# TheCacophonyProject/classifier-pipeline

Hardware: AMD Instinct MI355X
Metric: CPTV frames/s end-to-end (track+classify) at 160x120 (higher is better)
Workload: dtype u16/i32 track stage (f32 normalise, f64 gates); f32 crop/tile; f32 CNN (stride-1 3x3 convs of stages 2-4 (+ the stride-2 one): two fp16 planes per operand rounded to nearest (11 + 11 significand bits), power-of-two range scaling, 3 fp16 MFMAs per K step, device-side rerun in the exact split if an ac

## Files before the change

### classifier-pipeline_amd/csrc/cpx_api.cpp

```cpp
#include <hip/hip_runtime.h>

#include <algorithm>
#include <cmath>
#include <cstdio>
#include <cstdlib>
#include <cstring>
#include <new>
#include <string>
#include <vector>

#include "cpx_internal.h"
#include "cpx_schedule_core.h"

static_assert(sizeof(cpx_component) == 32, "cpx_component layout is part of the ABI");
static_assert(sizeof(cpx_frame_info) == 80, "cpx_frame_info layout is part of the ABI");
static_assert(sizeof(cpx_frame_meta) == 24, "cpx_frame_meta layout is part of the ABI");
static_assert(sizeof(cpx_config) == 48, "cpx_config layout is part of the ABI");
static_assert(sizeof(cpx_region_ref) == 24 && sizeof(cpx_track_limits) == 32 && sizeof(cpx_crop_req) == 32,
              "classification request layouts are part of the ABI");
static_assert(sizeof(cpx_filter_params) == 72 && sizeof(cpx_track_summary) == 120,
              "end-of-clip layouts are part of the ABI");
static_assert(sizeof(cpx_region) == 56, "cpx_region layout is part of the ABI");
static_assert(sizeof(cpx_track_record) == 32, "cpx_track_record layout is part of the ABI");
static_assert(sizeof(cpx_track_params) == 120, "cpx_track_params layout is part of the ABI");
// ... 100 lines not shown
    }
    if (lut[63] != 0 || h->nlm_lut_dev.grow(h, 64 * sizeof(int), "NLM weight table allocation") ||
        hipMemcpy(h->nlm_lut_dev.p, lut.data(), 64 * sizeof(int), hipMemcpyHostToDevice) != hipSuccess) {
      cpx_destroy(h);
      return CPX_ERR_HIP;
    }
  }
  std::vector<uint32_t> thr(h->wtab_len);
  for (int k = 0; k < h->wtab_len; ++k) {
    const double wk = wt[k], m = std::nearbyint(wk);
    const bool exact = (wk == m), near = !exact && std::fabs(wk - m) < 1e-6;
    double hi = near ? m + 1.0 : std::floor(wk) + 1.0;
    if (!(hi >= 0.0)) hi = 0.0;
    if (hi > 536870912.0) hi = 536870912.0;
    thr[k] = 2u * (uint32_t)hi - (near ? 1u : 0u);
  }
  if (h->wthr_dev.grow(h, thr.size() * sizeof(uint32_t), "threshold table allocation") ||
      hipMemcpy(h->wthr_dev.p, thr.data(), thr.size() * sizeof(uint32_t), hipMemcpyHostToDevice) != hipSuccess) {
    cpx_destroy(h);
    return CPX_ERR_HIP;
  }
  if (h->wtab_dev.grow(h, wt.size() * sizeof(double), "weight table allocation") ||
      hipMemcpy(h->wtab_dev.p, wt.data(), wt.size() * sizeof(double), hipMemcpyHostToDevice) != hipSuccess ||
      cpx::frame_kernel_attr_setup() != 0) {
    cpx_destroy(h);
    return CPX_ERR_HIP;
  }
  if (const char* env = std::getenv("CPX_TRACK_PACKED_STATE")) h->packed_state_ok = std::atoi(env) != 0;
  if (const char* env = std::getenv("CPX_CNN_FUSE_CONV1")) h->fuse_conv1 = std::atoi(env) != 0;
  if (const char* env = std::getenv("CPX_TRACK_PER_STEP")) h->track_per_step = std::atoi(env) != 0;
  if (const char* env = std::getenv("CPX_CNN_FUSE_SHORTCUT")) h->fuse_shortcut = std::atoi(env) != 0;
  if (const char* env = std::getenv("CPX_CNN_SHORTCUT_FP16")) h->shortcut_fp16 = std::atoi(env) != 0;
  if (const char* env = std::getenv("CPX_CNN_FLAT16")) h->flat16 = std::atoi(env) != 0;
  if (const char* env = std::getenv("CPX_CNN_BLOCK_FUSION")) h->block_fusion = std::min(std::max(std::atoi(env), 0), 2);
  if (const char* env = std::getenv("CPX_CNN_MATH")) {
    if (!std::strcmp(env, "f32")) h->cnn_math = CPX_CNN_MATH_F32;
    else if (!std::strcmp(env, "bf16x3")) h->cnn_math = CPX_CNN_MATH_BF16X3;
    else if (!std::strcmp(env, "bf16x2")) h->cnn_math = CPX_CNN_MATH_BF16X2;
    else if (!std::strcmp(env, "fp16x2")) h->cnn_math = CPX_CNN_MATH_FP16X2;
  }
  *out = h;
  return CPX_OK;
}

static void release_buffers(cpx_handle* h, bool all) {
  for (DeviceBuffer* b : {&h->ws, &h->ws_assoc, &h->bf3_scratch, &h->cnn_arena, &h->graph_arena, &h->ir_scratch}) b->release();
  if (!all) return;
  for (DeviceBuffer* b : {&h->sched, &h->wtab_dev, &h->wthr_dev, &h->nlm_lut_dev, &h->cnn_ovf, &h->ir_bitmap}) b->release();
}

void cpx_destroy(cpx_handle* h) {
  if (!h) return;
  hipSetDevice(h->device);
  if (h->stream) hipStreamSynchronize(h->stream);
  for (cpx_cnn* c : h->cnns) cnn_free(c);
  h->cnns.clear();
  for (cpx_mog2* m : h->mog2s) mog2_free(m);
  h->mog2s.clear();
  for (cpx_graph* g : h->graphs) graph_free(g);
  h->graphs.clear();
  release_buffers(h, true);
  for (auto& e : h->conv_events) {
    hipEventDestroy(e.e0);
    hipEventDestroy(e.e1);
  }
  if (h->stream2) {
// ... 731 lines not shown
```

### classifier-pipeline_amd/csrc/cpx_api_cnn.cpp

```cpp
#include <hip/hip_runtime.h>

#include <algorithm>
#include <cmath>
#include <cstdio>
#include <cstdlib>
#include <new>
#include <utility>
#include <vector>

#include "cpx_internal.h"

static_assert(sizeof(cpx_wrresnet_block) == 56 && sizeof(cpx_wrresnet_params) == 1560,
              "cpx_wrresnet_params layout is part of the ABI");

struct cpx_cnn {
  cpx_handle* h = nullptr;
  cpx_wrresnet_params p{};
  std::vector<std::pair<const float*, void*>> split;
  float act_scale[3][CPX_WRRESNET_MAX_BLOCKS][2];
  float res_bound[3] = {0.0f, 0.0f, 0.0f};
  float sc_xscale[3] = {0.0f, 0.0f, 0.0f};
  void* sc_img[3] = {nullptr, nullptr, nullptr};
  double sc_wmax[3] = {-1.0, -1.0, -1.0};
  cpx_cnn() {
// ... 123 lines not shown
  const conv_half& k = hf ? *hf : bare;
  const bool fp16 = split && h->cnn_math == CPX_CNN_MATH_FP16X2;
  const bool aliased = a.out == a.residual || a.out == a.in;
  const bool half = fp16 && cpx::conv_bf3_two_planes(a) && !aliased;
  const bool planes_out = fp16 && k.out_planes;
  const ConvRoute route = k.rerun_only ? ConvRoute::RerunOnly
                          : !split ? ConvRoute::Float32
                          : (half || planes_out) ? ConvRoute::Fp16Pair
                                                 : ConvRoute::Split;
  ConvTimer timer(h, h->conv_timing && route != ConvRoute::RerunOnly);
  if (!timer.ok()) return fail(h, CPX_ERR_HIP, "cpx_conv2d: event creation failed");
  int* word = nullptr;
  if (route == ConvRoute::Fp16Pair || route == ConvRoute::RerunOnly) {
    if (int rc = ensure_ovf_word(h)) return rc;
    if (!k.keep_flag) CPX_HIP(h, hipMemsetAsync(h->cnn_ovf.p, 0, sizeof(int), h->stream));
    word = h->cnn_ovf.as<int>() + k.word;
  }
  if (split && !split_weights) {
    if (int rc = h->bf3_scratch.grow(h, cpx::conv_bf3_weight_bytes(a), "cpx_conv2d: weight scratch allocation failed"))
      return rc;
    cpx::launch_split_weights(a, h->bf3_scratch.p, h->stream);
    split_weights = h->bf3_scratch.p;
  }
  int rc = 0;
  if (route == ConvRoute::Fp16Pair) {
    cpx::ConvArgs first = a;
    if (half) {
      first.planes = 2;
      first.half = 1;
      first.act_scale = k.act_scale;
      first.act_unscale = 1.0f / first.act_scale;
      first.in_planes = k.in_planes;
      first.flat16 = h->flat16;
    }
    first.ovf = word;
    if (planes_out) {
      first.out_planes = 1;
      first.out_act_scale = k.out_act_scale;
    }
    rc = cpx::launch_conv_bf3(first, split_weights, h->stream);
  }
  a.guard = word;
  if (split) {
    if (rc == 0) rc = cpx::launch_conv_bf3(a, split_weights, h->stream);
    if (rc == -3) {
      if (fuse) return fail(h, CPX_ERR_UNSUPPORTED, "conv_run: batch too large for the fused-shortcut kernel (split the call)");
      rc = cpx::launch_conv(a, h->stream);
    }
  } else {
    rc = cpx::launch_conv(a, h->stream);
  }
  if (int trc = timer.commit((a.Cin / a.groups) * 10000 + (a.Cout / a.groups) * 10 + a.stride + (a.ksize == 1 ? 5 : 0),
                             2.0 * a.N * a.Ho * a.Wo * a.Cout * (double)(a.Cin / a.groups) * a.ksize * a.ksize))
    return trc;
  if (rc == -2) return fail(h, CPX_ERR_UNSUPPORTED, "cpx_conv2d: no kernel for this (channels per group, stride, kernel size)");
  if (rc != 0) return fail(h, CPX_ERR_HIP, "cpx_conv2d: kernel configuration failed");
  CPX_HIP(h, hipGetLastError());
  return CPX_OK;
}

static bool conv_can_fuse(const cpx_handle* h, int f, int groups) {
  return split_math(h) && cpx::conv_bf3_supported(conv_shape(0, 0, 0, f, f, groups, 3, 1, 1));
}

enum class BlockForm {
  OneLaunch,
// ... 557 lines not shown
```

### classifier-pipeline_amd/csrc/cpx_cnn_rw.hip

```cpp
#include <hip/hip_runtime.h>

#include <algorithm>
#include <type_traits>

#include "cpx_cnn_dev.h"
#include "cpx_conv_layout_core.h"
#include "cpx_kernels.h"

namespace cpx {

namespace {

struct RwTiles : Tiles {};

constexpr int RW_TW = 16;
constexpr int RW_CT = 256;
constexpr int RW_PPI = RW_CT / 8;
constexpr int RW_WC = 64;

template <int S, int NCH, int ROWS>
struct RwGeo {
  static constexpr int PW = 15 * S + 3, PH = (ROWS - 1) * S + 3, NPX = PH * PW;
  static constexpr int NP = (NPX * 8 + RW_CT - 1) / RW_CT;
  static constexpr int NPXP = (NP * RW_PPI + 3) / 4 * 4 + 2;
  static constexpr int BUF = 2 * 2 * NPXP * 2;
  static constexpr int STEPS = 3 * PH;
  static constexpr int CING = 32 * NCH;
  static constexpr size_t LDS = (size_t)2 * BUF * 16 + (size_t)(2 * CING + 3 * RW_WC) * sizeof(float);
};
constexpr int SC_NPXP = 258;
constexpr int SC_ITEMS = 16 * RW_TW * 8 / RW_CT;
constexpr size_t SC_LDS = (size_t)2 * 2 * SC_NPXP * 2 * 16;

template <int S, int NCH, int ROWS, bool BN, bool RES, bool SC = false>
__global__ __launch_bounds__(RW_CT) __attribute__((amdgpu_waves_per_eu(1, 1))) void conv_rw_kernel(ConvArgs a, const uint4* __restrict__ wimg, RwTiles td) {
  using G = RwGeo<S, NCH, ROWS>;
  constexpr int PW = G::PW, NPX = G::NPX, NP = G::NP, NPXP = G::NPXP, BUF = G::BUF, STEPS = G::STEPS, CING = G::CING, PH = G::PH;
  static_assert(!SC || (S == 1 && NCH == 2 && ROWS == 16 && !RES), "the fp16 shortcut is built into the stride-1 form's two-chunk stream");
  if (*a.ovf != 0) return;
  extern __shared__ __attribute__((aligned(16))) uint4 lds4[];
  uint4* s_buf = lds4;
  float* s_bn = reinterpret_cast<float*>(lds4 + 2 * BUF);
  float* s_par = s_bn + 2 * CING;
  uint4* s_sc = reinterpret_cast<uint4*>(s_par + 3 * RW_WC);
  const int tid = threadIdx.x, lane = tid & 63, wave = tid >> 6, i16 = lane & 15, q = lane >> 4;
  const int ct = wave;
  const int cout_g = a.Cout / a.groups, nhalf = cout_g / RW_WC;
  const int g = blockIdx.y / nhalf, half = blockIdx.y - g * nhalf;
  constexpr bool has_bn = BN;

  u32x4 Wr[NCH][9][2];
  {
    const u32x4* wg = reinterpret_cast<const u32x4*>(wimg) + (size_t)g * NCH * 3 * 24 * cout_g + (q * cout_g + half * RW_WC + ct * 16 + i16);
#pragma unroll
    for (int c = 0; c < NCH; ++c)
#pragma unroll
      for (int ky = 0; ky < 3; ++ky)
#pragma unroll
        for (int kx = 0; kx < 3; ++kx)
#pragma unroll
          for (int p = 0; p < 2; ++p) Wr[c][ky * 3 + kx][p] = wg[(size_t)((c * 3 + ky) * 24 + (p * 3 + kx) * 4) * cout_g];
  }
  u32x4 Wsc[2];
  if constexpr (SC) {
    const u32x4* ws = reinterpret_cast<const u32x4*>(a.sc_planes) + (size_t)g * 8 * cout_g + (q * cout_g + half * RW_WC + ct * 16 + i16);
    Wsc[0] = ws[0];
    Wsc[1] = ws[(size_t)4 * cout_g];
  }
  if (tid < CING) {
    const int ci = g * CING + tid;
    s_bn[tid] = has_bn ? a.in_scale[ci] * a.act_scale : a.act_scale;
    s_bn[CING + tid] = has_bn ? a.in_shift[ci] * a.act_scale : 0.0f;
  }
  if (tid < RW_WC) {
    const int ch = g * cout_g + half * RW_WC + tid;
    float os = a.w_unscale[ch] * a.act_unscale;
    if (a.out_scale) os *= a.out_scale[ch];
    float ob = a.out_shift ? a.out_shift[ch] : 0.0f;
    if (a.sc_in && a.sc_bias) ob += a.sc_bias[ch];
    s_par[tid] = os;
    s_par[RW_WC + tid] = ob;
    s_par[2 * RW_WC + tid] = a.w_scale[ch] * a.act_scale;
  }

  const int per_xcd = (td.total + 7) >> 3;
  auto tile_of = [&](int t) { return (t & 7) * per_xcd + (t >> 3); };
  auto decode = [&](int tile, int& n_, int& oy_, int& ox_) {
    int qd = tile_div(tile, td.m_tx);
    ox_ = (tile - qd * td.tiles_x) * RW_TW;
    tile = qd;
    qd = tile_div(tile, td.m_ty);
    oy_ = (tile - qd * td.tiles_y) * ROWS;
    n_ = qd;
  };
  int t = blockIdx.x;
  while (t < 8 * per_xcd && tile_of(t) >= td.total) t += gridDim.x;
  if (t >= 8 * per_xcd) return;
  auto advance = [&](int& n_, int& oy_, int& ox_) {
    t += gridDim.x;
    const bool more = t < 8 * per_xcd && tile_of(t) < td.total;
    if (more) decode(tile_of(t), n_, oy_, ox_);
    return more;
  };
  int n0, oy0, ox0, n1, oy1, ox1, n2, oy2, ox2;
  decode(tile_of(t), n0, oy0, ox0);

  u32x4 pre_p[NP];
  const int q8 = tid & 7;
  int ipos[NP];
#pragma unroll
  for (int i = 0; i < NP; ++i) {
    const int px = min((tid >> 3) + RW_PPI * i, NPX - 1);
    const int py = px / PW;
    ipos[i] = (py << 8) | (px - py * PW);
  }
  const unsigned st_base = (unsigned)((((q8 >> 2) * NPXP + (tid >> 3)) * 4 + (q8 & 3)) * 8);
  f32x4 psc[NCH], psh[NCH];
  const unsigned coff0 = (unsigned)(g * CING + 4 * q8);
  const int Hm1 = a.H - 1, Wm1 = a.W - 1;
  auto issue_item = [&](const int i, const int c, const int n_, const int oy_, const int ox_) __attribute__((always_inline)) {
    const float* in_n = a.in + (size_t)n_ * a.H * a.W * a.Cin;
    const int iy = oy_ * S - a.pad_top + (ipos[i] >> 8), ix = ox_ * S - a.pad_left + (ipos[i] & 0xFF);
    const int cy = med3(iy, 0, Hm1), cx = med3(ix, 0, Wm1);
    pre_p[i] = *reinterpret_cast<const u32x4*>(at_off(in_n, (pix_off(cy, cx, a.W, a.Cin) + coff0 + (unsigned)(c * 32)) << 2));
  };
  unsigned hmax = 0u;
  auto activate_item = [&](const int i, const int c, const int oy_, const int ox_) __attribute__((always_inline)) {
    float v[4];
#pragma unroll
    for (int j = 0; j < 4; ++j) v[j] = __fmaf_rn(__uint_as_float(pre_p[i][j]), psc[c][j], psh[c][j]);
    if (has_bn) {
#pragma unroll
      for (int j = 0; j < 4; ++j) v[j] = fmaxf(v[j], 0.0f);
    }
    const int iy = oy_ * S - a.pad_top + (ipos[i] >> 8), ix = ox_ * S - a.pad_left + (ipos[i] & 0xFF);
    const bool inside = (unsigned)iy < (unsigned)a.H && (unsigned)ix < (unsigned)a.W;
#pragma unroll
    for (int j = 0; j < 4; ++j) pre_p[i][j] = __float_as_uint(inside ? v[j] : 0.0f);
  };
  auto store_item = [&](const int i, const int bsel) __attribute__((always_inline)) {
    unsigned h0, h1, l0, l1;
    split_pair2_h(__uint_as_float(pre_p[i][0]), __uint_as_float(pre_p[i][1]), h0, l0);
    split_pair2_h(__uint_as_float(pre_p[i][2]), __uint_as_float(pre_p[i][3]), h1, l1);
    if (has_bn) hmax = pk_max_u16(pk_max_u16(hmax, h0), h1);
    else hmax = pk_max_u16(pk_max_u16(hmax, h0 & 0x7FFF7FFFu), h1 & 0x7FFF7FFFu);
    unsigned char* sp = reinterpret_cast<unsigned char*>(s_buf) + st_base;
    *reinterpret_cast<uint2*>(sp + (bsel * BUF * 16 + i * (RW_PPI * 32))) = make_uint2(h0, h1);
    *reinterpret_cast<uint2*>(sp + (bsel * BUF * 16 + 2 * NPXP * 32 + i * (RW_PPI * 32))) = make_uint2(l0, l1);
  };

  u32x4 pre_s[SC ? SC_ITEMS : 1];
  u32x4 xsh[2], xsl[2];
  const unsigned sc_st_base = (unsigned)((((q8 >> 2) * SC_NPXP + (tid >> 3)) * 4 + (q8 & 3)) * 8);
  const int sc_a_base = ((q >> 1) * SC_NPXP + i16) * 2 + (q & 1);
  auto issue_sc = [&](const int i, const int n_, const int oy_, const int ox_) __attribute__((always_inline)) {
    if constexpr (SC) {
      const float* sc_n = a.sc_in + (size_t)n_ * a.sc_H * a.sc_W * a.sc_cin;
      const int oy = min(oy_ + 2 * i + (tid >> 7), a.Ho - 1), ox = min(ox_ + ((tid >> 3) & 15), a.Wo - 1);
      pre_s[i] = *reinterpret_cast<const u32x4*>(
          at_off(sc_n, (pix_off(oy * a.sc_stride, ox * a.sc_stride, a.sc_W, a.sc_cin) + (unsigned)(g * 32 + 4 * q8)) << 2));
    }
  };
  auto store_sc = [&](const int i) __attribute__((always_inline)) {
    if constexpr (SC) {
      unsigned h0, h1, l0, l1;
      split_pair2_h(__uint_as_float(pre_s[i][0]) * a.sc_xscale, __uint_as_float(pre_s[i][1]) * a.sc_xscale, h0, l0);
      split_pair2_h(__uint_as_float(pre_s[i][2]) * a.sc_xscale, __uint_as_float(pre_s[i][3]) * a.sc_xscale, h1, l1);
      hmax = pk_max_u16(pk_max_u16(hmax, h0 & 0x7FFF7FFFu), h1 & 0x7FFF7FFFu);
      unsigned char* sp = reinterpret_cast<unsigned char*>(s_sc) + sc_st_base;
      *reinterpret_cast<uint2*>(sp + i * (RW_PPI * 32)) = make_uint2(h0, h1);
      *reinterpret_cast<uint2*>(sp + (2 * SC_NPXP * 32 + i * (RW_PPI * 32))) = make_uint2(l0, l1);
    }
  };

  f32x4 acc[ROWS];
  const int ch_l = g * cout_g + half * RW_WC + ct * 16 + 4 * q;
  auto init_acc = [&]() __attribute__((always_inline)) {
#pragma unroll
    for (int o = 0; o < ROWS; ++o) acc[o] = f32x4{0.0f, 0.0f, 0.0f, 0.0f};
  };
  f32x4 rres[RES ? ROWS : 1];
  auto issue_res = [&](const int o, const int n_, const int oy_, const int ox_) __attribute__((always_inline)) {
    if constexpr (RES) {
      const float* res_n = a.residual + (size_t)n_ * a.Ho * a.Wo * a.Cout;
      const int ox = min(ox_ + i16, a.Wo - 1), oy = min(oy_ + o, a.Ho - 1);
      rres[o] = *reinterpret_cast<const f32x4*>(at_off(res_n, (pix_off(oy, ox, a.Wo, a.Cout) + (unsigned)ch_l) << 2));
    }
  };

  const int a_base = ((q >> 1) * NPXP + S * i16) * 2 + (q & 1);
  constexpr int RW_AHEAD = 3, RW_RING = RW_AHEAD + 1;
  auto compute = [&](auto cc, auto bc, auto&& between) __attribute__((always_inline)) {
    constexpr int C = decltype(cc)::value, B = decltype(bc)::value;
    const uint4* sb = s_buf + B * BUF + a_base;
    u32x4 xh[RW_RING], xl[RW_RING];
    auto frag = [&](auto sc) __attribute__((always_inline)) {
      constexpr int s = decltype(sc)::value;
      constexpr int kx = s / PH, i = s - PH * kx, bf = s % RW_RING;
      xh[bf] = __builtin_bit_cast(u32x4, sb[(i * PW + kx) * 2]);
      xl[bf] = __builtin_bit_cast(u32x4, sb[4 * NPXP + (i * PW + kx) * 2]);
    };
    static_for<0, RW_AHEAD>(frag);
    static_for<0, STEPS>([&](auto sc) __attribute__((always_inline)) {
      constexpr int s = decltype(sc)::value;
      constexpr int kx = s / PH, i = s - PH * kx, bf = s % RW_RING;
      if constexpr (s + RW_AHEAD < STEPS) frag(std::integral_constant<int, s + RW_AHEAD>{});
      static_for<0, 3>([&](auto pc) __attribute__((always_inline)) {
        constexpr int pr = decltype(pc)::value;
        static_for<0, 3>([&](auto rc) __attribute__((always_inline)) {
          constexpr int r = decltype(rc)::value, d = i - r, o = d / S;
          if constexpr (d >= 0 && d % S == 0 && o < ROWS) {
            if constexpr (pr == 0) acc[o] = mfma16<true>(Wr[C][r * 3 + kx][1], xh[bf], acc[o]);
            if constexpr (pr == 1) acc[o] = mfma16<true>(Wr[C][r * 3 + kx][0], xl[bf], acc[o]);
            if constexpr (pr == 2) acc[o] = mfma16<true>(Wr[C][r * 3 + kx][0], xh[bf], acc[o]);
          }
        });
      });
      between(sc);
      __builtin_amdgcn_sched_barrier(0);
    });
  };
  auto unit = [&](auto cc, auto bc, auto ccc, auto cic, auto lastc, const int oyc, const int oxc, const int ni, const int oyi,
                  const int oxi) __attribute__((always_inline)) {
    constexpr int B = decltype(bc)::value, CC = decltype(ccc)::value, CI = decltype(cic)::value;
    constexpr bool LAST = decltype(lastc)::value;
    compute(cc, bc, [&](auto sc) __attribute__((always_inline)) {
      constexpr int s = decltype(sc)::value;
      constexpr int jlo = (s * 3 * NP + STEPS - 1) / STEPS, jhi = ((s + 1) * 3 * NP + STEPS - 1) / STEPS;
      static_for<jlo, (jhi < 3 * NP ? jhi : 3 * NP)>([&](auto jc) __attribute__((always_inline)) {
        constexpr int j = decltype(jc)::value, i = j / 3, k = j % 3;
        if constexpr (k == 0) activate_item(i, CC, oyc, oxc);
        if constexpr (k == 1) store_item(i, B ^ 1);
        if constexpr (k == 2) issue_item(i, CI, ni, oyi, oxi);
      });
      if constexpr (SC && !LAST) {
        constexpr int klo = (s * SC_ITEMS + STEPS - 1) / STEPS, khi = ((s + 1) * SC_ITEMS + STEPS - 1) / STEPS;
        static_for<klo, (khi < SC_ITEMS ? khi : SC_ITEMS)>([&](auto kc) __attribute__((always_inline)) { store_sc(decltype(kc)::value); });
      }
      if constexpr (SC && LAST) {
        if constexpr (s % 3 == 0 && s >= 3 && s / 3 - 1 < ROWS) {
          constexpr int o = s / 3 - 1;
          acc[o] = mfma16<true>(Wsc[1], xsh[o & 1], acc[o]);
          acc[o] = mfma16<true>(Wsc[0], xsl[o & 1], acc[o]);
          acc[o] = mfma16<true>(Wsc[0], xsh[o & 1], acc[o]);
        }
        if constexpr (s % 3 == 0 && s / 3 < ROWS) {
          constexpr int o = s / 3;
          xsh[o & 1] = __builtin_bit_cast(u32x4, s_sc[sc_a_base + o * 2 * RW_TW]);
          xsl[o & 1] = __builtin_bit_cast(u32x4, s_sc[sc_a_base + 4 * SC_NPXP + o * 2 * RW_TW]);
        }
        constexpr int klo = (s * SC_ITEMS + STEPS - 1) / STEPS, khi = ((s + 1) * SC_ITEMS + STEPS - 1) / STEPS;
        static_for<klo, (khi < SC_ITEMS ? khi : SC_ITEMS)>([&](auto kc) __attribute__((always_inline)) { issue_sc(decltype(kc)::value, ni, oyi, oxi); });
      }
      if constexpr (LAST && RES) {
        constexpr int olo = (s * ROWS + STEPS - 1) / STEPS, ohi = ((s + 1) * ROWS + STEPS - 1) / STEPS;
        static_for<olo, (ohi < ROWS ? ohi : ROWS)>([&](auto oc) __attribute__((always_inline)) { issue_res(decltype(oc)::value, n0, oy0, ox0); });
      }
    });
  };

  auto finish = [&](const int n_, const int oy_, const int ox_) __attribute__((always_inline)) {
    const int ox = min(ox_ + i16, a.Wo - 1);
    if (!SC && a.sc_in) {
      const int sc_cg = a.sc_cin / a.groups;
      const float* wsc = a.sc_w + ((size_t)g * sc_cg + q) * cout_g + half * RW_WC + ct * 16 + i16;
      const float ss = s_par[2 * RW_WC + ct * 16 + i16];
      const float* sc_n = a.sc_in + (size_t)n_ * a.sc_H * a.sc_W * a.sc_cin + g * sc_cg + q;
      for (int k4 = 0; k4 < sc_cg; k4 += 4) {
        const float ws = wsc[(size_t)k4 * cout_g] * ss;
#pragma unroll
        for (int o = 0; o < ROWS; ++o) {
          const int oy = min(oy_ + o, a.Ho - 1);
          const float xs = sc_n[((size_t)(oy * a.sc_stride) * a.sc_W + ox * a.sc_stride) * a.sc_cin + k4];
          acc[o] = __builtin_amdgcn_mfma_f32_16x16x4f32(ws, xs, acc[o], 0, 0, 0);
        }
      }
    }
    float* out_n = a.out + (size_t)n_ * a.Ho * a.Wo * a.Cout;
    const f32x4 os = *reinterpret_cast<const f32x4*>(s_par + ct * 16 + 4 * q);
    const f32x4 ob = *reinterpret_cast<const f32x4*>(s_par + RW_WC + ct * 16 + 4 * q);
    const bool xok = ox_ + i16 < a.Wo;
    const unsigned off0 = (pix_off(min(oy_, a.Ho - 1), ox, a.Wo, a.Cout) + (unsigned)ch_l) << 2;
    const unsigned row_bytes = (unsigned)(a.Wo * a.Cout) << 2;
    const bool whole = oy_ + ROWS <= a.Ho;
    auto row = [&](const int o, const bool ok, const unsigned off) __attribute__((always_inline)) {
      f32x4 v;
#pragma unroll
      for (int j = 0; j < 4; ++j) v[j] = __fmaf_rn(acc[o][j], os[j], ob[j]);
      if constexpr (RES) v += rres[o];
      if (a.relu) {
        asm volatile("");
        v.x = relu_bits(v.x); v.y = relu_bits(v.y); v.z = relu_bits(v.z); v.w = relu_bits(v.w);
      }
      if (ok) *reinterpret_cast<f32x4*>(at_off(out_n, off)) = v;
    };
    if (whole) {
#pragma unroll
      for (int o = 0; o < ROWS; ++o) row(o, xok, off0 + (unsigned)o * row_bytes);
    } else {
#pragma unroll
      for (int o = 0; o < ROWS; ++o) row(o, xok && oy_ + o < a.Ho, off0 + (unsigned)min(o, a.Ho - 1 - oy_) * row_bytes);
    }
  };

#pragma unroll
  for (int i = 0; i < NP; ++i) issue_item(i, 0, n0, oy0, ox0);
  __syncthreads();
#pragma unroll
  for (int c = 0; c < NCH; ++c) {
    psc[c] = *reinterpret_cast<const f32x4*>(s_bn + c * 32 + 4 * q8);
    psh[c] = *reinterpret_cast<const f32x4*>(s_bn + CING + c * 32 + 4 * q8);
  }
#pragma unroll
  for (int i = 0; i < NP; ++i) {
    activate_item(i, 0, oy0, ox0);
    store_item(i, 0);
  }
  using I0 = std::integral_constant<int, 0>;
  using I1 = std::integral_constant<int, 1>;
  using Yes = std::integral_constant<bool, true>;
  using No = std::integral_constant<bool, false>;
  if constexpr (NCH == 2) {
#pragma unroll
    for (int i = 0; i < NP; ++i) issue_item(i, 1, n0, oy0, ox0);
    if constexpr (SC) {
#pragma unroll
      for (int i = 0; i < SC_ITEMS; ++i) issue_sc(i, n0, oy0, ox0);
    }
    init_acc();
    for (;;) {
      n1 = n0; oy1 = oy0; ox1 = ox0;
      const bool more = advance(n1, oy1, ox1);
      __syncthreads();
      unit(I0{}, I0{}, I1{}, I0{}, No{}, oy0, ox0, n1, oy1, ox1);
      __syncthreads();
      unit(I1{}, I1{}, I0{}, I1{}, Yes{}, oy1, ox1, n1, oy1, ox1);
      finish(n0, oy0, ox0);
      if (!more) break;
      n0 = n1; oy0 = oy1; ox0 = ox1;
      init_acc();
    }
  } else {
    n1 = n0; oy1 = oy0; ox1 = ox0;
    bool more1 = advance(n1, oy1, ox1);
#pragma unroll
    for (int i = 0; i < NP; ++i) issue_item(i, 0, n1, oy1, ox1);
    init_acc();
    for (;;) {
      n2 = n1; oy2 = oy1; ox2 = ox1;
      bool more2 = more1 && advance(n2, oy2, ox2);
      __syncthreads();
      unit(I0{}, I0{}, I0{}, I0{}, Yes{}, oy1, ox1, n2, oy2, ox2);
      finish(n0, oy0, ox0);
      if (!more1) break;
      n0 = n1; oy0 = oy1; ox0 = ox1; n1 = n2; oy1 = oy2; ox1 = ox2; more1 = more2;
// ... 25 lines not shown
  const float f = wscale[g * cout_g + col] * factor;
  float v[8];
#pragma unroll
  for (int j = 0; j < 8; ++j) v[j] = w[((size_t)g * cin_g + chunk * 32 + 8 * qq + j) * cout_g + col] * f;
  uint4 hi, lo;
  split_pair2_h(v[0], v[1], hi.x, lo.x);
  split_pair2_h(v[2], v[3], hi.y, lo.y);
  split_pair2_h(v[4], v[5], hi.z, lo.z);
  split_pair2_h(v[6], v[7], hi.w, lo.w);
  const size_t base = (size_t)(g * nch + chunk) * 8 * cout_g + (size_t)qq * cout_g + col;
  out[base] = hi;
  out[base + (size_t)4 * cout_g] = lo;
}

}

bool conv_shortcut_planes_layer(const ConvArgs& second, int sc_cin_g) {
  if (conv_rw_kind(second) == 1) return sc_cin_g == 32;
  return second.ksize == 3 && second.stride == 1 && second.groups >= 1 && second.Cin == second.Cout &&
         second.Cout == 128 * second.groups && sc_cin_g == 64;
}
size_t conv_shortcut_image_bytes(int groups, int cin_g, int cout_g) { return (size_t)groups * (cin_g / 32) * 8 * cout_g * 16; }
void launch_split_shortcut(const float* sc_w, void* img, int groups, int cin_g, int cout_g, const float* w_scale, float factor,
                           hipStream_t s) {
  const int total = groups * (cin_g / 32) * 4 * cout_g;
  hipLaunchKernelGGL(split_shortcut_kernel, dim3((unsigned)((total + 255) / 256)), dim3(256), 0, s, sc_w, reinterpret_cast<uint4*>(img),
                     groups, cin_g, cout_g, w_scale, factor);
}

int conv_rw_kind(const ConvArgs& a) { return conv_rw_kind_of(conv_shape_of(a)); }
bool conv_rw_layer(const ConvArgs& a) { return conv_rw_kind(a) == 1; }

namespace {
template <int S, int NCH, int ROWS, bool BN, bool RES, bool SC = false>
int launch_rw_t(const ConvArgs& a, const uint4* wimg, hipStream_t s) {
  using G = RwGeo<S, NCH, ROWS>;
  constexpr size_t LDS = G::LDS + (SC ? SC_LDS : 0);
  static_assert(LDS <= 160 * 1024 - 1024, "two chunk buffers (and the shortcut's operand) must fit the CU's LDS");
  RwTiles td{};
  if (const int rc = fill_tiles(td, (a.Wo + RW_TW - 1) / RW_TW, (a.Ho + ROWS - 1) / ROWS, a.N, TILES_PERSISTENT)) return rc;
  static bool lds_ready[64];
  if (!cpx_dyn_lds_ready(reinterpret_cast<const void*>(conv_rw_kernel<S, NCH, ROWS, BN, RES, SC>), lds_ready, 160 * 1024 - 1024)) return -1;
  const int ny = a.groups * ((a.Cout / a.groups) / RW_WC);
  const int gx = persistent_grid(cpx_device_cus(), ny, td.total);
  if (gx < 0) return -1;
  hipLaunchKernelGGL((conv_rw_kernel<S, NCH, ROWS, BN, RES, SC>), dim3((unsigned)gx, (unsigned)ny), dim3(RW_CT), LDS, s, a, wimg, td);
  return 0;
}
}

int launch_conv_rw(const ConvArgs& a, const void* wimg, hipStream_t s) {
  const int kind = conv_rw_kind(a);
  if (!kind || !a.half || a.planes != 2 || a.ovf == nullptr || a.in_planes || a.out_planes) return -2;
  if ((long long)a.H * a.W >= (1 << 24) || (long long)a.Ho * a.Wo >= (1 << 24)) return -3;
  if (a.sc_in && ((a.sc_cin / a.groups) & 3)) return -2;
  const uint4* wi = reinterpret_cast<const uint4*>(wimg);
  const bool bn = a.in_scale != nullptr, res = a.residual != nullptr;
  if (kind == 1) {
    if (a.pad_top != 1 || a.pad_left != 1 || a.H != a.Ho || a.W != a.Wo) return -2;
    if (a.sc_in && a.sc_planes) {
      if (bn || res || !conv_shortcut_planes_layer(a, a.sc_cin / a.groups) || a.sc_stride < 1 || !(a.sc_xscale > 0.0f) ||
          (a.sc_H - 1) / a.sc_stride + 1 != a.Ho || (a.sc_W - 1) / a.sc_stride + 1 != a.Wo)
        return -2;
      if ((long long)a.sc_H * a.sc_W >= (1 << 24) || (long long)a.sc_H * a.sc_W * a.sc_cin >= (1ll << 30)) return -3;
      return launch_rw_t<1, 2, 16, false, false, true>(a, wi, s);
    }
    if (bn && res) return launch_rw_t<1, 2, 16, true, true>(a, wi, s);
    if (bn) return launch_rw_t<1, 2, 16, true, false>(a, wi, s);
    if (res) return launch_rw_t<1, 2, 16, false, true>(a, wi, s);
    return launch_rw_t<1, 2, 16, false, false>(a, wi, s);
  }
  if (res || a.sc_in || a.pad_top < 0 || a.pad_top > 1 || a.pad_left < 0 || a.pad_left > 1) return -2;
  if (kind == 2) return bn ? launch_rw_t<2, 1, 8, true, false>(a, wi, s) : launch_rw_t<2, 1, 8, false, false>(a, wi, s);
  return bn ? launch_rw_t<3, 2, 4, true, false>(a, wi, s) : launch_rw_t<3, 2, 4, false, false>(a, wi, s);
}

}
```

### classifier-pipeline_amd/csrc/cpx_conv_layout_core.h

```cpp
#pragma once
#include <stddef.h>
#include <stdlib.h>

#include <algorithm>

namespace cpx {

struct ConvShape { int groups, cin_g, cout_g, ksize, stride; };
template <class Args>
ConvShape conv_shape_of(const Args& a) {
  if (a.groups < 1 || a.Cin % a.groups || a.Cout % a.groups) return ConvShape{};
  return ConvShape{a.groups, a.Cin / a.groups, a.Cout / a.groups, a.ksize, a.stride};
}

enum class ConvClass { Unsupported, Plain, Flat, Wide, C8, Stride2Rw, Rw3 };

inline ConvClass conv_class(const ConvShape& s) {
  if (s.ksize != 3) return ConvClass::Unsupported;
  if (s.stride == 3 && s.cin_g == 64 && s.cout_g == 128) return ConvClass::Rw3;
  if (s.stride == 2 && s.cin_g == 32 && s.cout_g == 64) return ConvClass::Stride2Rw;
  if (s.stride == 1 && s.cin_g == 8 && s.cout_g == 32) return ConvClass::C8;
  const bool c32_64 = s.cout_g == 32 || s.cout_g == 64;
  if (s.stride == 1 && (s.cin_g == 32 || s.cin_g == 64) && c32_64) return ConvClass::Wide;
  if (s.cin_g < 16 || s.cin_g % 16) return ConvClass::Unsupported;
// ... 58 lines not shown
}
struct Tiles {
  unsigned long long m_tx, m_ty;
  int tiles_x, tiles_y, total;
};

template <class T>
int fill_tiles(T& td, int tiles_x, int tiles_y, long long n, long long limit) {
  if (tiles_x < 1 || tiles_y < 1 || tiles_x >= TILE_AXIS_LIMIT || tiles_y >= TILE_AXIS_LIMIT) return -3;
  const long long total = (long long)tiles_x * tiles_y * n;
  if (total >= limit) return -3;
  td.tiles_x = tiles_x, td.m_tx = tile_magic(tiles_x);
  td.tiles_y = tiles_y, td.m_ty = tile_magic(tiles_y);
  td.total = (int)total;
  return 0;
}
template <class T>
int fill_tiles(T& td, int tiles_x, int tiles_y, long long n, int nsplit, long long limit) {
  if (nsplit < 1 || nsplit >= TILE_AXIS_LIMIT) return -3;
  td.nsplit = nsplit, td.m_nsplit = tile_magic(nsplit);
  return fill_tiles(td, tiles_x, tiles_y, n * nsplit, limit);
}

inline int persistent_grid_x(int cus, int ny, long long tiles) {
  const int gx = std::max(8, cus / std::max(ny, 1) / 8 * 8);
  return (int)std::min<long long>(gx, (tiles + 7) / 8 * 8);
}
inline int persistent_grid(int cus, int ny, long long tiles, const char* width_env = nullptr) {
  if (cus == 0) return -1;
  const char* e = width_env ? getenv(width_env) : nullptr;
  return e ? persistent_grid_x(atoi(e), 1, tiles) : persistent_grid_x(cus, ny, tiles);
}

enum { WALK_TILES = 0, WALK_ROWS = 1 };
struct BlkTiles {
  unsigned long long m_tx, m_ty;
  int tiles_x, tiles_y, total;
  int walk, units;
};
static_assert(sizeof(BlkTiles) == 40 && offsetof(BlkTiles, total) == offsetof(Tiles, total) && offsetof(BlkTiles, walk) == 28 &&
                  offsetof(BlkTiles, units) == 32,
              "the argument layout conv_block32s_kernel was tuned with");
inline void set_walk(BlkTiles& td, int walk) {
  td.walk = walk;
  td.units = walk == WALK_ROWS ? td.total / td.tiles_x : td.total;
}
CPX_WALK_HD bool walk_tile(const BlkTiles& td, int bx, int gx, int j, int& n, int& ty, int& tx) {
  int col = 0;
  if (td.walk == WALK_ROWS) {
    const int jr = tile_div(j, td.m_tx);
    col = j - jr * td.tiles_x;
    j = jr;
  }
  const int per_xcd = (td.units + 7) >> 3;
  const int t = bx + j * gx;
  if (t >= 8 * per_xcd) return false;
  int unit = (t & 7) * per_xcd + (t >> 3);
  if (unit >= td.units) return false;
  if (td.walk == WALK_ROWS) {
    tx = td.tiles_x - 1 - col;
  } else {
    const int qd = tile_div(unit, td.m_tx);
    tx = unit - qd * td.tiles_x;
    unit = qd;
  }
  n = tile_div(unit, td.m_ty);
// ... 16 lines not shown
```

### classifier-pipeline_amd/csrc/cpx_internal.h

```cpp
#pragma once
#include <hip/hip_runtime.h>

#include <map>
#include <string>
#include <vector>

#include "cpx.h"
#include "cpx_kernels.h"

struct cpx_cnn;
struct cpx_mog2;
struct cpx_graph;
void cnn_free(cpx_cnn* c);
void graph_free(cpx_graph* g);
void mog2_free(cpx_mog2* m);

struct DeviceBuffer {
  void* p = nullptr;
  size_t bytes = 0;
  DeviceBuffer() = default;
  DeviceBuffer(const DeviceBuffer&) = delete;
  DeviceBuffer& operator=(const DeviceBuffer&) = delete;
  int grow(cpx_handle* h, size_t need, const char* what);
  void release() {
// ... 14 lines not shown
  DeviceBuffer wtab_dev, wthr_dev;
  int wtab_len = 0;
  std::vector<double> wtab_host;
  DeviceBuffer nlm_lut_dev;
  DeviceBuffer sched;
  struct ConvEv { int key; double flops; hipEvent_t e0, e1; };
  std::vector<ConvEv> conv_events;
  bool conv_timing = false;
  DeviceBuffer ws_assoc;
  hipEvent_t ev0 = nullptr, ev1 = nullptr;
  int last_launches = 0;
  bool timing_valid = false;
  hipStream_t stream2 = nullptr;
  bool state_packed = false;
  bool packed_state_ok = true;
  bool fuse_conv1 = true;
  bool medians_pending = false;
  hipEvent_t ev_median = nullptr;
  bool track_per_step = false;
  std::vector<struct cpx_cnn*> cnns;
  std::vector<struct cpx_mog2*> mog2s;
  std::vector<struct cpx_graph*> graphs;
  DeviceBuffer graph_arena;
  int stream_frames = -1;
  int stream_assoc_frames = -1;
  bool stream_filt_state = false;
  int last_B = 0;
  struct StagedBackground { std::vector<uint16_t> bg, kcnt; double average; };
  std::map<int, StagedBackground> staged_bg;
  int cnn_math = CPX_CNN_MATH_FP16X2;
  bool fuse_shortcut = true;
  bool shortcut_fp16 = true;
  bool flat16 = true;
  DeviceBuffer bf3_scratch;
  DeviceBuffer cnn_arena;
  DeviceBuffer cnn_ovf;
  int block_fusion = 2;
  DeviceBuffer ir_scratch;
  DeviceBuffer ir_bitmap;
};

inline int fail(cpx_handle* h, int code, const char* what, hipError_t e = hipSuccess) {
  if (h) {
    h->err = what;
    if (e != hipSuccess) {
      h->err += ": ";
      h->err += hipGetErrorString(e);
    }
  }
  return code;
}

#define CPX_HIP(h, call)                                            \
  do {                                                              \
    hipError_t _e = (call);                                         \
    if (_e != hipSuccess) return fail((h), CPX_ERR_HIP, #call, _e); \
  } while (0)

#define CPX_ENTER(h)                           \
  do {                                         \
    CPX_HIP((h), hipSetDevice((h)->device));   \
    (void)hipGetLastError();                   \
  } while (0)

inline int DeviceBuffer::grow(cpx_handle* h, size_t need, const char* what) {
  if (need <= bytes) return CPX_OK;
// ... 14 lines not shown
```

### classifier-pipeline_amd/csrc/cpx_kernels.h

```cpp
#pragma once
#include <hip/hip_runtime.h>
#include <stddef.h>
#include <stdint.h>

#include "cpx.h"

#ifndef CPX_TRACK_THREADS
#define CPX_TRACK_THREADS 768
#endif
#ifndef CPX_TRACK_CHUNKS
#define CPX_TRACK_CHUNKS 7
#endif
#ifndef CPX_TRACK_LDS_COMPONENTS
#define CPX_TRACK_LDS_COMPONENTS 256
#endif
#ifndef CPX_TRACK_MIN_WAVES_PER_SIMD
#define CPX_TRACK_MIN_WAVES_PER_SIMD 6
#endif

namespace cpx {

typedef cpx_component Component;
typedef cpx_frame_info FrameInfo;

// ... 133 lines not shown
void launch_aggregate(const AggregateArgs& a, hipStream_t s);
void launch_limits(const ClassifyArgs& a, int n_tracks, hipStream_t s);
int launch_crop(const ClassifyArgs& a, int n_reqs, hipStream_t s);

struct ConvArgs {
  int N, H, W, Cin, Cout, groups, ksize, stride, relu;
  int Ho, Wo, pad_top, pad_left;
  const float* in;
  float* out;
  const float* weights;
  const float* in_scale;
  const float* in_shift;
  const float* out_scale;
  const float* out_shift;
  const float* residual;
  const float* sc_in;
  const float* sc_w;
  const float* sc_bias;
  int sc_H, sc_W, sc_cin, sc_stride;
  const void* sc_planes;
  float sc_xscale;
  const float* c1_in;
  const float* c1_w;
  const float* c1_b;
  int planes;
  int half;
  float act_scale, act_unscale;
  const float* w_scale;
  const float* w_unscale;
  int* ovf;
  const int* guard;
  int out_planes, in_planes;
  float out_act_scale;
  int flat16;
};
static_assert(sizeof(ConvArgs) == 264, "the argument layout the convolution kernels were tuned with");
struct HeadArgs {
  int N, HW, C, L;
  int n_hidden, activation;
  int hidden_sizes[CPX_HEAD_MAX_HIDDEN];
  const float* in;
  const float* bn_scale;
  const float* bn_shift;
  const float* hidden_w[CPX_HEAD_MAX_HIDDEN];
  const float* hidden_b[CPX_HEAD_MAX_HIDDEN];
  const float* dense_w;
  const float* dense_b;
  float* logits;
  float* probs;
};
int launch_conv(const ConvArgs& a, hipStream_t s);
bool conv_bf3_supported(const ConvArgs& a);
size_t conv_bf3_weight_bytes(const ConvArgs& a);
bool conv_bf3_two_planes(const ConvArgs& a);
bool conv_bf3_can_store_planes(const ConvArgs& a);
bool conv_bf3_can_load_planes(const ConvArgs& a);
void launch_split_weights(const ConvArgs& a, void* wimg, hipStream_t s);
int launch_conv_bf3(const ConvArgs& a, const void* wimg, hipStream_t s);
bool conv_block32_supported(const ConvArgs& a, const ConvArgs& b);
int launch_conv_block32(const ConvArgs& a, const ConvArgs& b, const void* wimg_a, const void* wimg_b, hipStream_t s);
int launch_conv_block32s(const ConvArgs& a, const ConvArgs& b, const void* wa, const void* wb, hipStream_t s);
int conv_rw_kind(const ConvArgs& a);
bool conv_rw_layer(const ConvArgs& a);
int launch_conv_rw(const ConvArgs& a, const void* wimg, hipStream_t s);
int launch_conv_flat16(const ConvArgs& a, const void* wimg, hipStream_t s);
bool conv_shortcut_planes_layer(const ConvArgs& second, int sc_cin_g);
size_t conv_shortcut_image_bytes(int groups, int cin_g, int cout_g);
// ... 181 lines not shown
```

Baseline: 3.232 million.

## Split input-channel chunks of stride-1 fp16 conv across paired wave sets

Adds a paired variant of the row-wise stride-1 fp16-pair convolution kernel. Each block now runs two 256-thread wave sets, and each set handles one of the two 32-channel input chunks with its own LDS staging buffers. The second set parks its partial accumulators in LDS and the first set adds them during the epilogue. Tiles shrink to 8 rows and the weight registers per thread are halved, aiming for more parallelism and two waves per EU instead of one long serial chunk loop. In exchange it adds a cross-set reduction through LDS, extra barriers, and more LDS per block. It is enabled by default through a new rw_pair flag that can be turned off with an environment variable.

```diff
diff --git a/classifier-pipeline_amd/csrc/cpx_api.cpp b/classifier-pipeline_amd/csrc/cpx_api.cpp
--- a/classifier-pipeline_amd/csrc/cpx_api.cpp
+++ b/classifier-pipeline_amd/csrc/cpx_api.cpp
@@ -156,6 +156,7 @@
   if (const char* env = std::getenv("CPX_CNN_FUSE_SHORTCUT")) h->fuse_shortcut = std::atoi(env) != 0;
   if (const char* env = std::getenv("CPX_CNN_SHORTCUT_FP16")) h->shortcut_fp16 = std::atoi(env) != 0;
   if (const char* env = std::getenv("CPX_CNN_FLAT16")) h->flat16 = std::atoi(env) != 0;
+  if (const char* env = std::getenv("CPX_CNN_RW_PAIR")) h->rw_pair = std::atoi(env) != 0;
   if (const char* env = std::getenv("CPX_CNN_BLOCK_FUSION")) h->block_fusion = std::min(std::max(std::atoi(env), 0), 2);
   if (const char* env = std::getenv("CPX_CNN_MATH")) {
     if (!std::strcmp(env, "f32")) h->cnn_math = CPX_CNN_MATH_F32;
diff --git a/classifier-pipeline_amd/csrc/cpx_api_cnn.cpp b/classifier-pipeline_amd/csrc/cpx_api_cnn.cpp
--- a/classifier-pipeline_amd/csrc/cpx_api_cnn.cpp
+++ b/classifier-pipeline_amd/csrc/cpx_api_cnn.cpp
@@ -179,6 +179,7 @@
       first.act_unscale = 1.0f / first.act_scale;
       first.in_planes = k.in_planes;
       first.flat16 = h->flat16;
+      first.rw_pair = h->rw_pair;
     }
     first.ovf = word;
     if (planes_out) {
diff --git a/classifier-pipeline_amd/csrc/cpx_cnn_rw.hip b/classifier-pipeline_amd/csrc/cpx_cnn_rw.hip
--- a/classifier-pipeline_amd/csrc/cpx_cnn_rw.hip
+++ b/classifier-pipeline_amd/csrc/cpx_cnn_rw.hip
@@ -13,47 +13,39 @@
 
 struct RwTiles : Tiles {};
 
-constexpr int RW_TW = 16;
-constexpr int RW_CT = 256;
-constexpr int RW_PPI = RW_CT / 8;
-constexpr int RW_WC = 64;
-
-template <int S, int NCH, int ROWS>
-struct RwGeo {
-  static constexpr int PW = 15 * S + 3, PH = (ROWS - 1) * S + 3, NPX = PH * PW;
-  static constexpr int NP = (NPX * 8 + RW_CT - 1) / RW_CT;
-  static constexpr int NPXP = (NP * RW_PPI + 3) / 4 * 4 + 2;
-  static constexpr int BUF = 2 * 2 * NPXP * 2;
-  static constexpr int STEPS = 3 * PH;
-  static constexpr int CING = 32 * NCH;
-  static constexpr size_t LDS = (size_t)2 * BUF * 16 + (size_t)(2 * CING + 3 * RW_WC) * sizeof(float);
-};
+constexpr int RW_CT = RW_SET;
 constexpr int SC_NPXP = 258;
 constexpr int SC_ITEMS = 16 * RW_TW * 8 / RW_CT;
 constexpr size_t SC_LDS = (size_t)2 * 2 * SC_NPXP * 2 * 16;
 
-template <int S, int NCH, int ROWS, bool BN, bool RES, bool SC = false>
-__global__ __launch_bounds__(RW_CT) __attribute__((amdgpu_waves_per_eu(1, 1))) void conv_rw_kernel(ConvArgs a, const uint4* __restrict__ wimg, RwTiles td) {
-  using G = RwGeo<S, NCH, ROWS>;
-  constexpr int PW = G::PW, NPX = G::NPX, NP = G::NP, NPXP = G::NPXP, BUF = G::BUF, STEPS = G::STEPS, CING = G::CING, PH = G::PH;
-  static_assert(!SC || (S == 1 && NCH == 2 && ROWS == 16 && !RES), "the fp16 shortcut is built into the stride-1 form's two-chunk stream");
+template <int S, int NCH, int ROWS, bool BN, bool RES, bool SC = false, bool PAIR = false>
+__global__ __launch_bounds__((PAIR ? NCH : 1) * RW_SET) __attribute__((amdgpu_waves_per_eu(PAIR ? 2 : 1, PAIR ? 2 : 1))) void conv_rw_kernel(ConvArgs a, const uint4* __restrict__ wimg, RwTiles td) {
+  using G = RwGeo<S, NCH, ROWS, PAIR>;
+  constexpr int PW = G::PW, NP = G::NP, NPXP = G::NPXP, BUF = G::BUF, STEPS = G::STEPS, CING = G::CING, PH = G::PH;
+  constexpr int KC = PAIR ? 1 : NCH;
+  static_assert(!SC || (S == 1 && NCH == 2 && ROWS == 16 && !RES && !PAIR), "the fp16 shortcut is built into the stride-1 form's two-chunk stream");
+  static_assert(!PAIR || (S == 1 && NCH == 2), "the paired form: two chunks, two wave sets");
+  static_assert(!G::CLAMPED || (NP - 1) * RW_PPI <= NPXP, "only the last staging item's slot may need the clamp");
   if (*a.ovf != 0) return;
   extern __shared__ __attribute__((aligned(16))) uint4 lds4[];
   uint4* s_buf = lds4;
-  float* s_bn = reinterpret_cast<float*>(lds4 + 2 * BUF);
+  float* s_bn = reinterpret_cast<float*>(lds4 + G::NBUF * BUF);
   float* s_par = s_bn + 2 * CING;
   uint4* s_sc = reinterpret_cast<uint4*>(s_par + 3 * RW_WC);
+  f32x4* s_red = reinterpret_cast<f32x4*>(s_par + 3 * RW_WC);
   const int tid = threadIdx.x, lane = tid & 63, wave = tid >> 6, i16 = lane & 15, q = lane >> 4;
-  const int ct = wave;
+  const int ct = PAIR ? wave & 3 : wave;
+  const int cw = PAIR ? __builtin_amdgcn_readfirstlane(wave >> 2) : 0;
+  const int ts = PAIR ? tid & (RW_SET - 1) : tid;
   const int cout_g = a.Cout / a.groups, nhalf = cout_g / RW_WC;
   const int g = blockIdx.y / nhalf, half = blockIdx.y - g * nhalf;
   constexpr bool has_bn = BN;
 
-  u32x4 Wr[NCH][9][2];
+  u32x4 Wr[KC][9][2];
   {
-    const u32x4* wg = reinterpret_cast<const u32x4*>(wimg) + (size_t)g * NCH * 3 * 24 * cout_g + (q * cout_g + half * RW_WC + ct * 16 + i16);
-#pragma unroll
-    for (int c = 0; c < NCH; ++c)
+    const u32x4* wg = reinterpret_cast<const u32x4*>(wimg) + (size_t)g * NCH * 3 * 24 * cout_g + (size_t)(cw * 3 * 24) * cout_g + (q * cout_g + half * RW_WC + ct * 16 + i16);
+#pragma unroll
+    for (int c = 0; c < KC; ++c)
 #pragma unroll
       for (int ky = 0; ky < 3; ++ky)
 #pragma unroll
@@ -85,14 +77,7 @@
 
   const int per_xcd = (td.total + 7) >> 3;
   auto tile_of = [&](int t) { return (t & 7) * per_xcd + (t >> 3); };
-  auto decode = [&](int tile, int& n_, int& oy_, int& ox_) {
-    int qd = tile_div(tile, td.m_tx);
-    ox_ = (tile - qd * td.tiles_x) * RW_TW;
-    tile = qd;
-    qd = tile_div(tile, td.m_ty);
-    oy_ = (tile - qd * td.tiles_y) * ROWS;
-    n_ = qd;
-  };
+  auto decode = [&](int tile, int& n_, int& oy_, int& ox_) { rw_tile_origin(td, tile, ROWS, n_, oy_, ox_); };
   int t = blockIdx.x;
   while (t < 8 * per_xcd && tile_of(t) >= td.total) t += gridDim.x;
   if (t >= 8 * per_xcd) return;
@@ -106,17 +91,18 @@
   decode(tile_of(t), n0, oy0, ox0);
 
   u32x4 pre_p[NP];
-  const int q8 = tid & 7;
+  const int q8 = ts & 7;
   int ipos[NP];
 #pragma unroll
   for (int i = 0; i < NP; ++i) {
-    const int px = min((tid >> 3) + RW_PPI * i, NPX - 1);
+    const int px = G::item_pixel(ts, i);
     const int py = px / PW;
     ipos[i] = (py << 8) | (px - py * PW);
   }
-  const unsigned st_base = (unsigned)((((q8 >> 2) * NPXP + (tid >> 3)) * 4 + (q8 & 3)) * 8);
-  f32x4 psc[NCH], psh[NCH];
-  const unsigned coff0 = (unsigned)(g * CING + 4 * q8);
+  const unsigned st_base = G::item_byte(ts, 0) + (unsigned)(cw * BUF * 16);
+  const unsigned st_last = G::item_byte(ts, NP - 1) + (unsigned)(cw * BUF * 16);
+  f32x4 psc[KC], psh[KC];
+  const unsigned coff0 = (unsigned)(g * CING + cw * 32 + 4 * q8);
   const int Hm1 = a.H - 1, Wm1 = a.W - 1;
   auto issue_item = [&](const int i, const int c, const int n_, const int oy_, const int ox_) __attribute__((always_inline)) {
     const float* in_n = a.in + (size_t)n_ * a.H * a.W * a.Cin;
@@ -144,14 +130,16 @@
     split_pair2_h(__uint_as_float(pre_p[i][2]), __uint_as_float(pre_p[i][3]), h1, l1);
     if (has_bn) hmax = pk_max_u16(pk_max_u16(hmax, h0), h1);
     else hmax = pk_max_u16(pk_max_u16(hmax, h0 & 0x7FFF7FFFu), h1 & 0x7FFF7FFFu);
-    unsigned char* sp = reinterpret_cast<unsigned char*>(s_buf) + st_base;
-    *reinterpret_cast<uint2*>(sp + (bsel * BUF * 16 + i * (RW_PPI * 32))) = make_uint2(h0, h1);
-    *reinterpret_cast<uint2*>(sp + (bsel * BUF * 16 + 2 * NPXP * 32 + i * (RW_PPI * 32))) = make_uint2(l0, l1);
+    const bool clamped = G::CLAMPED && i == NP - 1;
+    unsigned char* sp = reinterpret_cast<unsigned char*>(s_buf) + (clamped ? st_last : st_base);
+    const int at = bsel * G::BSTRIDE * 16 + (clamped ? 0 : i * (RW_PPI * 32));
+    *reinterpret_cast<uint2*>(sp + at) = make_uint2(h0, h1);
+    *reinterpret_cast<uint2*>(sp + (at + 2 * NPXP * 32)) = make_uint2(l0, l1);
   };
 
   u32x4 pre_s[SC ? SC_ITEMS : 1];
   u32x4 xsh[2], xsl[2];
-  const unsigned sc_st_base = (unsigned)((((q8 >> 2) * SC_NPXP + (tid >> 3)) * 4 + (q8 & 3)) * 8);
+  const unsigned sc_st_base = (unsigned)((((q8 >> 2) * SC_NPXP + (ts >> 3)) * 4 + (q8 & 3)) * 8);
   const int sc_a_base = ((q >> 1) * SC_NPXP + i16) * 2 + (q & 1);
   auto issue_sc = [&](const int i, const int n_, const int oy_, const int ox_) __attribute__((always_inline)) {
     if constexpr (SC) {
@@ -182,17 +170,18 @@
   f32x4 rres[RES ? ROWS : 1];
   auto issue_res = [&](const int o, const int n_, const int oy_, const int ox_) __attribute__((always_inline)) {
     if constexpr (RES) {
+      if (cw != 0) return;
       const float* res_n = a.residual + (size_t)n_ * a.Ho * a.Wo * a.Cout;
       const int ox = min(ox_ + i16, a.Wo - 1), oy = min(oy_ + o, a.Ho - 1);
       rres[o] = *reinterpret_cast<const f32x4*>(at_off(res_n, (pix_off(oy, ox, a.Wo, a.Cout) + (unsigned)ch_l) << 2));
     }
   };
 
-  const int a_base = ((q >> 1) * NPXP + S * i16) * 2 + (q & 1);
-  constexpr int RW_AHEAD = 3, RW_RING = RW_AHEAD + 1;
+  const int a_base = ((q >> 1) * NPXP + S * i16) * 2 + (q & 1) + cw * BUF;
+  constexpr int RW_AHEAD = PAIR ? 2 : 3, RW_RING = RW_AHEAD + 1;
   auto compute = [&](auto cc, auto bc, auto&& between) __attribute__((always_inline)) {
     constexpr int C = decltype(cc)::value, B = decltype(bc)::value;
-    const uint4* sb = s_buf + B * BUF + a_base;
+    const uint4* sb = s_buf + B * G::BSTRIDE + a_base;
     u32x4 xh[RW_RING], xl[RW_RING];
     auto frag = [&](auto sc) __attribute__((always_inline)) {
       constexpr int s = decltype(sc)::value;
@@ -259,9 +248,20 @@
     });
   };
 
-  auto finish = [&](const int n_, const int oy_, const int ox_) __attribute__((always_inline)) {
+  auto park = [&](const int par) __attribute__((always_inline)) {
+    f32x4* r = s_red + ((par * 4 + ct) * ROWS) * 64 + lane;
+#pragma unroll
+    for (int o = 0; o < ROWS; ++o) r[o * 64] = acc[o];
+  };
+
+  auto finish = [&](const int n_, const int oy_, const int ox_, const int par = 0) __attribute__((always_inline)) {
     const int ox = min(ox_ + i16, a.Wo - 1);
-    if (!SC && a.sc_in) {
+    if constexpr (PAIR) {
+      const f32x4* r = s_red + ((par * 4 + ct) * ROWS) * 64 + lane;
+#pragma unroll
+      for (int o = 0; o < ROWS; ++o) acc[o] = acc[o] + r[o * 64];
+    }
+    if (!SC && !PAIR && a.sc_in) {
       const int sc_cg = a.sc_cin / a.groups;
       const float* wsc = a.sc_w + ((size_t)g * sc_cg + q) * cout_g + half * RW_WC + ct * 16 + i16;
       const float ss = s_par[2 * RW_WC + ct * 16 + i16];
@@ -307,9 +307,9 @@
   for (int i = 0; i < NP; ++i) issue_item(i, 0, n0, oy0, ox0);
   __syncthreads();
 #pragma unroll
-  for (int c = 0; c < NCH; ++c) {
-    psc[c] = *reinterpret_cast<const f32x4*>(s_bn + c * 32 + 4 * q8);
-    psh[c] = *reinterpret_cast<const f32x4*>(s_bn + CING + c * 32 + 4 * q8);
+  for (int c = 0; c < KC; ++c) {
+    psc[c] = *reinterpret_cast<const f32x4*>(s_bn + (c + cw) * 32 + 4 * q8);
+    psh[c] = *reinterpret_cast<const f32x4*>(s_bn + CING + (c + cw) * 32 + 4 * q8);
   }
 #pragma unroll
   for (int i = 0; i < NP; ++i) {
@@ -320,7 +320,31 @@
   using I1 = std::integral_constant<int, 1>;
   using Yes = std::integral_constant<bool, true>;
   using No = std::integral_constant<bool, false>;
-  if constexpr (NCH == 2) {
+  if constexpr (PAIR) {
+    n1 = n0; oy1 = oy0; ox1 = ox0;
+    bool more1 = advance(n1, oy1, ox1);
+#pragma unroll
+    for (int i = 0; i < NP; ++i) issue_item(i, 0, n1, oy1, ox1);
+    int np = 0, oyp = 0, oxp = 0, parp = -1;
+    auto tile = [&](auto bc) __attribute__((always_inline)) {
+      constexpr int B = decltype(bc)::value;
+      n2 = n1; oy2 = oy1; ox2 = ox1;
+      const bool more2 = more1 && advance(n2, oy2, ox2);
+      __syncthreads();
+      if (cw == 0 && parp >= 0) finish(np, oyp, oxp, parp);
+      init_acc();
+      unit(I0{}, bc, I0{}, I0{}, Yes{}, oy1, ox1, n2, oy2, ox2);
+      if (cw != 0) park(B);
+      np = n0; oyp = oy0; oxp = ox0; parp = B;
+      const bool go = more1;
+      n0 = n1; oy0 = oy1; ox0 = ox1; n1 = n2; oy1 = oy2; ox1 = ox2; more1 = more2;
+      return go;
+    };
+    while (tile(I0{}) && tile(I1{})) {
+    }
+    __syncthreads();
+    if (cw == 0) finish(np, oyp, oxp, parp);
+  } else if constexpr (NCH == 2) {
 #pragma unroll
     for (int i = 0; i < NP; ++i) issue_item(i, 1, n0, oy0, ox0);
     if constexpr (SC) {
@@ -412,19 +436,19 @@
 bool conv_rw_layer(const ConvArgs& a) { return conv_rw_kind(a) == 1; }
 
 namespace {
-template <int S, int NCH, int ROWS, bool BN, bool RES, bool SC = false>
+template <int S, int NCH, int ROWS, bool BN, bool RES, bool SC = false, bool PAIR = false>
 int launch_rw_t(const ConvArgs& a, const uint4* wimg, hipStream_t s) {
-  using G = RwGeo<S, NCH, ROWS>;
+  using G = RwGeo<S, NCH, ROWS, PAIR>;
   constexpr size_t LDS = G::LDS + (SC ? SC_LDS : 0);
-  static_assert(LDS <= 160 * 1024 - 1024, "two chunk buffers (and the shortcut's operand) must fit the CU's LDS");
+  static_assert(LDS <= 160 * 1024 - 1024, "the chunk buffers (and the shortcut's operand or the pairs' scratch) must fit the CU's LDS");
   RwTiles td{};
-  if (const int rc = fill_tiles(td, (a.Wo + RW_TW - 1) / RW_TW, (a.Ho + ROWS - 1) / ROWS, a.N, TILES_PERSISTENT)) return rc;
+  if (const int rc = rw_fill_tiles(td, a.Wo, a.Ho, a.N, ROWS)) return rc;
   static bool lds_ready[64];
-  if (!cpx_dyn_lds_ready(reinterpret_cast<const void*>(conv_rw_kernel<S, NCH, ROWS, BN, RES, SC>), lds_ready, 160 * 1024 - 1024)) return -1;
+  if (!cpx_dyn_lds_ready(reinterpret_cast<const void*>(conv_rw_kernel<S, NCH, ROWS, BN, RES, SC, PAIR>), lds_ready, 160 * 1024 - 1024)) return -1;
   const int ny = a.groups * ((a.Cout / a.groups) / RW_WC);
   const int gx = persistent_grid(cpx_device_cus(), ny, td.total);
   if (gx < 0) return -1;
-  hipLaunchKernelGGL((conv_rw_kernel<S, NCH, ROWS, BN, RES, SC>), dim3((unsigned)gx, (unsigned)ny), dim3(RW_CT), LDS, s, a, wimg, td);
+  hipLaunchKernelGGL((conv_rw_kernel<S, NCH, ROWS, BN, RES, SC, PAIR>), dim3((unsigned)gx, (unsigned)ny), dim3(G::THREADS), LDS, s, a, wimg, td);
   return 0;
 }
 }
@@ -445,6 +469,13 @@
       if ((long long)a.sc_H * a.sc_W >= (1 << 24) || (long long)a.sc_H * a.sc_W * a.sc_cin >= (1ll << 30)) return -3;
       return launch_rw_t<1, 2, 16, false, false, true>(a, wi, s);
     }
+    if (a.rw_pair && !a.sc_in) {
+      constexpr int T = RW_PAIR_ROWS;
+      if (bn && res) return launch_rw_t<1, 2, T, true, true, false, true>(a, wi, s);
+      if (bn) return launch_rw_t<1, 2, T, true, false, false, true>(a, wi, s);
+      if (res) return launch_rw_t<1, 2, T, false, true, false, true>(a, wi, s);
+      return launch_rw_t<1, 2, T, false, false, false, true>(a, wi, s);
+    }
     if (bn && res) return launch_rw_t<1, 2, 16, true, true>(a, wi, s);
     if (bn) return launch_rw_t<1, 2, 16, true, false>(a, wi, s);
     if (res) return launch_rw_t<1, 2, 16, false, true>(a, wi, s);
diff --git a/classifier-pipeline_amd/csrc/cpx_conv_layout_core.h b/classifier-pipeline_amd/csrc/cpx_conv_layout_core.h
--- a/classifier-pipeline_amd/csrc/cpx_conv_layout_core.h
+++ b/classifier-pipeline_amd/csrc/cpx_conv_layout_core.h
@@ -114,6 +114,46 @@
   return e ? persistent_grid_x(atoi(e), 1, tiles) : persistent_grid_x(cus, ny, tiles);
 }
 
+constexpr int RW_TW = 16;
+constexpr int RW_SET = 256;
+constexpr int RW_PPI = RW_SET / 8;
+constexpr int RW_WC = 64;
+template <int S, int NCH, int ROWS, bool PAIR = false>
+struct RwGeo {
+  static constexpr int PW = 15 * S + 3, PH = (ROWS - 1) * S + 3, NPX = PH * PW;
+  static constexpr int NP = (NPX * 8 + RW_SET - 1) / RW_SET;
+  static constexpr int NPXP = PAIR ? (NPX + 3) / 4 * 4 + 2 : (NP * RW_PPI + 3) / 4 * 4 + 2;
+  static constexpr int BUF = 2 * 2 * NPXP * 2;
+  static constexpr int NBUF = PAIR ? 2 * NCH : 2;
+  static constexpr int BSTRIDE = (PAIR ? NCH : 1) * BUF;
+  static constexpr int STEPS = 3 * PH;
+  static constexpr int CING = 32 * NCH;
+  static constexpr int THREADS = PAIR ? NCH * RW_SET : RW_SET;
+  static constexpr int RED = PAIR ? 2 * 4 * ROWS * 64 : 0;
+  static constexpr size_t PARAMS = (size_t)(2 * CING + 3 * RW_WC) * sizeof(float);
+  static constexpr size_t LDS = (size_t)NBUF * BUF * 16 + PARAMS + (size_t)RED * 16;
+  static constexpr int item_pixel(int ts, int i) { return std::min((ts >> 3) + RW_PPI * i, NPX - 1); }
+  static constexpr int item_slot(int ts, int i) { return std::min((ts >> 3) + RW_PPI * i, NPXP - 1); }
+  static constexpr unsigned item_byte(int ts, int i) {
+    return (unsigned)(((((ts & 7) >> 2) * NPXP + item_slot(ts, i)) * 4 + (ts & 3)) * 8);
+  }
+  static constexpr bool CLAMPED = NP * RW_PPI > NPXP;
+};
+constexpr int RW_PAIR_ROWS = 8;
+template <class T>
+CPX_WALK_HD void rw_tile_origin(const T& td, int tile, int rows, int& n, int& oy, int& ox) {
+  int qd = tile_div(tile, td.m_tx);
+  ox = (tile - qd * td.tiles_x) * RW_TW;
+  tile = qd;
+  qd = tile_div(tile, td.m_ty);
+  oy = (tile - qd * td.tiles_y) * rows;
+  n = qd;
+}
+template <class T>
+int rw_fill_tiles(T& td, int Wo, int Ho, long long n, int rows) {
+  return fill_tiles(td, (Wo + RW_TW - 1) / RW_TW, (Ho + rows - 1) / rows, n, TILES_PERSISTENT);
+}
+
 enum { WALK_TILES = 0, WALK_ROWS = 1 };
 struct BlkTiles {
   unsigned long long m_tx, m_ty;
diff --git a/classifier-pipeline_amd/csrc/cpx_internal.h b/classifier-pipeline_amd/csrc/cpx_internal.h
--- a/classifier-pipeline_amd/csrc/cpx_internal.h
+++ b/classifier-pipeline_amd/csrc/cpx_internal.h
@@ -70,6 +70,7 @@
   bool fuse_shortcut = true;
   bool shortcut_fp16 = true;
   bool flat16 = true;
+  bool rw_pair = true;
   DeviceBuffer bf3_scratch;
   DeviceBuffer cnn_arena;
   DeviceBuffer cnn_ovf;
diff --git a/classifier-pipeline_amd/csrc/cpx_kernels.h b/classifier-pipeline_amd/csrc/cpx_kernels.h
--- a/classifier-pipeline_amd/csrc/cpx_kernels.h
+++ b/classifier-pipeline_amd/csrc/cpx_kernels.h
@@ -189,7 +189,7 @@
   const int* guard;
   int out_planes, in_planes;
   float out_act_scale;
-  int flat16;
+  short flat16, rw_pair;
 };
 static_assert(sizeof(ConvArgs) == 264, "the argument layout the convolution kernels were tuned with");
 struct HeadArgs {
```

Result: no change. 3.255 million (median of 5 runs) (+0.7%).
